# xiaosu-zhu/McQuic

Hardware: AMD Instinct MI355X
Metric: images/sec encode+decode, 768x512 Kodak-shape batch, qp=2 (higher is better)
Workload: dtype f32; 1 GPU; qp=2 reference model Compressor(128, 2, [8192, 2048, 512]), batch=32 768x512 random images per GPU, encode+decode tensor path (BASELINE configs[1]); images_per_gpu=32, parallelism=dp1 (independent image shards, no data-path collective)

## Files before the change

mcquic_amd/csrc/conv_mfma_kernel.h:

```cpp
#pragma once
#include <type_traits>

#include "mcq_common.h"
#include "../../include/mcquic_hip.h"

#ifndef MCQ_PF42A
#define MCQ_PF42A 9
#endif
#ifndef MCQ_PF42B
#define MCQ_PF42B 18
#endif
#ifndef MCQ_PFB
#define MCQ_PFB 18
#endif
#ifndef MCQ_WINO_PERSIST
#define MCQ_WINO_PERSIST 1
#endif
#ifndef MCQ_WINO_PFB2
#define MCQ_WINO_PFB2 48
#endif
#ifndef MCQ_CONV_MAX_MULTI
#define MCQ_CONV_MAX_MULTI 4
#endif

// ... 404 lines not shown
            if constexpr (POST == 2) {
                if (fl & MCQ_CONV_RESIDUAL) {
                    const __amdgpu_buffer_rsrc_t rr = mcq_make_rsrc(mcq_uniform_ptr(P_res + oslab), oslab_bytes);
                    float rv[2][16];
#pragma unroll
                    for (int r = 0; r < 16; ++r) rv[0][r] = mcq_buffer_load_s(rr, pvo, band_so(0, r));
#pragma unroll
                    for (int mb = 0; mb < 4; ++mb) {
                        if (mb < 3) {
#pragma unroll
                            for (int r = 0; r < 16; ++r) rv[(mb + 1) & 1][r] = mcq_buffer_load_s(rr, pvo, band_so(mb + 1, r));
                        }
#pragma unroll
                        for (int r = 0; r < 16; ++r) acc[mb][nb][r] = acc[mb][nb][r] + p.res_scale * rv[mb & 1][r];
                        __builtin_amdgcn_sched_barrier(0);
                    }
                }
            }
            f32x16 sacc[4];
#pragma unroll
            for (int q = 0; q < 4; ++q)
#pragma unroll
                for (int r = 0; r < 16; ++r) sacc[q][r] = mcq_buffer_load_s(pbr, (unsigned)hi * 16u, (unsigned)(q * 32 + mcq_drow(r, 0)) * 4u);
            f32x4v AP[POST_PF];
#pragma unroll
            for (int st = 0; st < POST_PF; ++st) AP[st] = mcq_wload<4>(pwr, pwlane, (unsigned)st * 1024u);
            __builtin_amdgcn_sched_barrier(0);
#pragma unroll
            for (int t = 0; t < POST_STEPS; ++t) {
                float b = acc[t >> 4][nb][t & 15];
                if (POST == 1) b = b * b;
#pragma unroll
                for (int q = 0; q < 4; ++q) sacc[q] = __builtin_amdgcn_mfma_f32_32x32x2f32(AP[t % POST_PF][q], b, sacc[q], 0, 0, 0);
                AP[t % POST_PF] = mcq_wload<4>(pwr, pwlane, (unsigned)(t + POST_PF) * 1024u);
                __builtin_amdgcn_sched_barrier(0);
            }
            if constexpr (POST == 1) {
#pragma unroll
                for (int q = 0; q < 4; ++q) {
                    if (fl & MCQ_CONV_POST_IGDN) {
#pragma unroll
                        for (int r = 0; r < 16; ++r) sacc[q][r] = acc[q][nb][r] * sqrtf(sacc[q][r]);
                    } else {
#pragma unroll
                        for (int r = 0; r < 16; ++r) sacc[q][r] = acc[q][nb][r] * (1.0f / sqrtf(sacc[q][r]));
                    }
#pragma unroll
                    for (int r = 0; r < 16; ++r) mcq_buffer_store_s(sacc[q][r], yr, pvo, band_so(q, r));
                    __builtin_amdgcn_sched_barrier(0);
                }
            } else {
                const __amdgpu_buffer_rsrc_t mr = mcq_make_rsrc(mcq_uniform_ptr(P_mul + oslab), oslab_bytes);
                const __amdgpu_buffer_rsrc_t gr = mcq_make_rsrc(mcq_uniform_ptr(P_gid + oslab), oslab_bytes);
                const __amdgpu_buffer_rsrc_t y2r = mcq_make_rsrc(mcq_uniform_ptr(((fl & MCQ_CONV_DUAL_SILU) ? P_y2 : P_y) + oslab), oslab_bytes);
                float m[2][16], gi[2][16];
#pragma unroll
                for (int r = 0; r < 16; ++r) { m[0][r] = mcq_buffer_load_s(mr, pvo, band_so(0, r)); gi[0][r] = mcq_buffer_load_s(gr, pvo, band_so(0, r)); }
#pragma unroll
                for (int q = 0; q < 4; ++q) {
                    if (q < 3) {
#pragma unroll
                        for (int r = 0; r < 16; ++r) {
                            m[(q + 1) & 1][r] = mcq_buffer_load_s(mr, pvo, band_so(q + 1, r));
                            gi[(q + 1) & 1][r] = mcq_buffer_load_s(gr, pvo, band_so(q + 1, r));
                        }
                    }
#pragma unroll
                    for (int r = 0; r < 16; ++r) sacc[q][r] = m[q & 1][r] * mcq_sigmoid(sacc[q][r]) + gi[q & 1][r];
#pragma unroll
                    for (int r = 0; r < 16; ++r) mcq_buffer_store_s(sacc[q][r], yr, pvo, band_so(q, r));
                    if (fl & MCQ_CONV_DUAL_SILU) {
#pragma unroll
                        for (int r = 0; r < 16; ++r) mcq_buffer_store_s(mcq_silu(sacc[q][r]), y2r, pvo, band_so(q, r));
                    }
                    __builtin_amdgcn_sched_barrier(0);
                }
            }
        }
        return;
    }
    const unsigned fl = p.flags;
    const unsigned HoWo = (unsigned)(p.Ho * p.Wo + tile_zero);
    const unsigned slab_bytes = (unsigned)p.Cout * HoWo * 4u;

    auto epilogue = [&](auto tag, const bool tile_active, auto&& get_acc, const int mb_first, auto count_tag) {
        constexpr unsigned EF = decltype(tag)::value;
        constexpr int MC = decltype(count_tag)::value;
        const unsigned f = EF == RUNTIME_FLAGS ? fl : EF;
        if (!tile_active) return;
        unsigned pvo[NB];
        __amdgpu_buffer_rsrc_t yr[NB], y2r[NB], rr_[NB], mr[NB], gr[NB];
#pragma unroll
        for (int nb = 0; nb < NB; ++nb) {
            const size_t slab = (size_t)img[nb] * p.Cout * HoWo;
            yr[nb] = mcq_make_rsrc(mcq_uniform_ptr(P_y + slab), slab_bytes);
            constexpr unsigned GBWD = MCQ_CONV_GDN_BWD | MCQ_CONV_IGDN_BWD | MCQ_CONV_GATE_BWD;
            if (f & (MCQ_CONV_DUAL_SILU | GBWD)) y2r[nb] = mcq_make_rsrc(mcq_uniform_ptr(P_y2 + slab), slab_bytes);
            if (f & (MCQ_CONV_RESIDUAL | GBWD)) rr_[nb] = mcq_make_rsrc(mcq_uniform_ptr(P_res + slab), slab_bytes);
            if (f & (MCQ_CONV_GDN | MCQ_CONV_IGDN | MCQ_CONV_GATE | MCQ_CONV_MUL | MCQ_CONV_DSILU_MUL | GBWD))
                mr[nb] = mcq_make_rsrc(mcq_uniform_ptr(P_mul + slab), slab_bytes);
            if (f & MCQ_CONV_GATE) gr[nb] = mcq_make_rsrc(mcq_uniform_ptr(P_gid + slab), slab_bytes);
            if (f & MCQ_CONV_SHUFFLE2)
                pvo[nb] = valid[nb] ? ((unsigned)hi * 4u * HoWo + (unsigned)(2 * yo[nb]) * (unsigned)(2 * p.Wo) + (unsigned)(2 * xo[nb])) * 4u
                                    : MCQ_OOB;
            else
                pvo[nb] = valid[nb] ? ((unsigned)(yo[nb] * p.Wo + xo[nb]) + 4u * (unsigned)hi * HoWo) * 4u : MCQ_OOB;
        }
        const __amdgpu_buffer_rsrc_t br = mcq_make_rsrc(mcq_uniform_ptr(P_bias ? P_bias : P_wp), P_bias ? (unsigned)p.Cout * 4u : 0u);

#pragma unroll
        for (int mi = 0; mi < MC; ++mi) {
            const int mb = mb_first + mi;
            const unsigned co_row0 = (unsigned)(co_base + mb * 32);
            float bias16[16];
#pragma unroll
            for (int r = 0; r < 16; ++r)
                bias16[r] = mcq_buffer_load_s(br, (unsigned)hi * 16u, (co_row0 + (unsigned)mcq_drow(r, 0)) * 4u);
            constexpr unsigned SIMPLE = MCQ_CONV_SILU_OUT | MCQ_CONV_RESIDUAL | MCQ_CONV_DUAL_SILU | MCQ_CONV_DSILU_MUL;
            if (EF != RUNTIME_FLAGS && (EF & ~SIMPLE) == 0u && NB <= 2) {
                unsigned sob[16];
#pragma unroll
                for (int r = 0; r < 16; ++r) sob[r] = (co_row0 + (unsigned)mcq_drow(r, 0)) * HoWo * 4u;
                constexpr int EB = OCC >= 3 ? 1 : NB;
#pragma unroll
                for (int nb0 = 0; nb0 < NB; nb0 += EB) {
                    float vv[EB][16], rvv[EB][16], tw[EB][16];
                    if (EF & MCQ_CONV_DSILU_MUL) {
                        if constexpr (PAIR && EB == 2) {
#pragma unroll
                            for (int r = 0; r < 16; ++r) { const f32x2v t2 = mcq_buffer_load2_s(mr[0], pvo[0], sob[r]); tw[0][r] = t2[0]; tw[1][r] = t2[1]; }
                        } else {
#pragma unroll
                        for (int e = 0; e < EB; ++e)
#pragma unroll
                            for (int r = 0; r < 16; ++r) tw[e][r] = mcq_buffer_load_s(mr[nb0 + e], pvo[nb0 + e], sob[r]);
                        }
                    }
                    if (EF & MCQ_CONV_RESIDUAL) {
                        if constexpr (PAIR && EB == 2) {
#pragma unroll
                            for (int r = 0; r < 16; ++r) { const f32x2v t2 = mcq_buffer_load2_s(rr_[0], pvo[0], sob[r]); rvv[0][r] = t2[0]; rvv[1][r] = t2[1]; }
                        } else {
#pragma unroll
                        for (int e = 0; e < EB; ++e)
#pragma unroll
                            for (int r = 0; r < 16; ++r) rvv[e][r] = mcq_buffer_load_s(rr_[nb0 + e], pvo[nb0 + e], sob[r]);
                        }
                    }
#pragma unroll
                    for (int e = 0; e < EB; ++e) {
                        get_acc(mi, nb0 + e, vv[e]);
#pragma unroll
                        for (int r = 0; r < 16; ++r) vv[e][r] = vv[e][r] + bias16[r];
                        if (EF & MCQ_CONV_DSILU_MUL) {
#pragma unroll
                            for (int r = 0; r < 16; ++r) vv[e][r] = vv[e][r] * mcq_dsilu(tw[e][r]);
                        }
                        if (EF & MCQ_CONV_RESIDUAL) {
#pragma unroll
                            for (int r = 0; r < 16; ++r) vv[e][r] = vv[e][r] + p.res_scale * rvv[e][r];
                        }
                        if (EF & MCQ_CONV_SILU_OUT) {
#pragma unroll
                            for (int r = 0; r < 16; ++r) vv[e][r] = mcq_silu(vv[e][r]);
                        }
                        if (EF & MCQ_CONV_DUAL_SILU) {
#pragma unroll
                            for (int r = 0; r < 16; ++r) tw[e][r] = mcq_silu(vv[e][r]);
                        }
                    }
                    if constexpr (PAIR && EB == 2) {
#pragma unroll
                        for (int r = 0; r < 16; ++r) mcq_buffer_store2_s(f32x2v{vv[0][r], vv[1][r]}, yr[0], pvo[0], sob[r]);
                        if (EF & MCQ_CONV_DUAL_SILU) {
#pragma unroll
                            for (int r = 0; r < 16; ++r) mcq_buffer_store2_s(f32x2v{tw[0][r], tw[1][r]}, y2r[0], pvo[0], sob[r]);
                        }
                    } else {
#pragma unroll
                    for (int e = 0; e < EB; ++e) {
#pragma unroll
                        for (int r = 0; r < 16; ++r) mcq_buffer_store_s(vv[e][r], yr[nb0 + e], pvo[nb0 + e], sob[r]);
                        if (EF & MCQ_CONV_DUAL_SILU) {
#pragma unroll
                            for (int r = 0; r < 16; ++r) mcq_buffer_store_s(tw[e][r], y2r[nb0 + e], pvo[nb0 + e], sob[r]);
                        }
                    }
                    }
                }
                continue;
            }
            if constexpr (PAIR) {
                float v0[16], v1[16];
                get_acc(mi, 0, v0);
                get_acc(mi, 1, v1);
#pragma unroll
                for (int r = 0; r < 16; ++r) { v0[r] = v0[r] + bias16[r]; v1[r] = v1[r] + bias16[r]; }
                if (f & MCQ_CONV_SHUFFLE2) {
                    const unsigned W2b = 2u * (unsigned)p.Wo * 4u;
#pragma unroll
                    for (int rq = 0; rq < 4; ++rq) {
                        const unsigned so = ((co_row0 >> 2) + 2u * (unsigned)rq) * HoWo * 16u;
                        f32x4v top = f32x4v{v0[rq * 4 + 0], v0[rq * 4 + 1], v1[rq * 4 + 0], v1[rq * 4 + 1]};
                        f32x4v bot = f32x4v{v0[rq * 4 + 2], v0[rq * 4 + 3], v1[rq * 4 + 2], v1[rq * 4 + 3]};
                        if (f & MCQ_CONV_DSILU_MUL) {
                            const f32x4v mt = mcq_buffer_load4_s(mr[0], pvo[0], so), mb2 = mcq_buffer_load4_s(mr[0], pvo[0], so + W2b);
#pragma unroll
                            for (int e = 0; e < 4; ++e) { top[e] = top[e] * mcq_dsilu(mt[e]); bot[e] = bot[e] * mcq_dsilu(mb2[e]); }
                        }
// ... 89 lines not shown
                    for (int r = 0; r < 16; ++r) {
                        const float sg = mcq_sigmoid(v[r]);
                        mcq_buffer_store_s(g[r] * sg, yr[nb], pvo[nb], so[r]);
                        mcq_buffer_store_s(g[r] * m[r] * sg * (1.0f - sg), y2r[nb], pvo[nb], so[r]);
                    }
                    continue;
                }
                if (f & (MCQ_CONV_GDN | MCQ_CONV_IGDN | MCQ_CONV_GATE | MCQ_CONV_MUL | MCQ_CONV_DSILU_MUL)) {
                    float m[16];
#pragma unroll
                    for (int r = 0; r < 16; ++r) m[r] = mcq_buffer_load_s(mr[nb], pvo[nb], so[r]);
                    if (f & MCQ_CONV_GDN) {
#pragma unroll
                        for (int r = 0; r < 16; ++r) v[r] = m[r] * (1.0f / sqrtf(v[r]));
                    } else if (f & MCQ_CONV_IGDN) {
#pragma unroll
                        for (int r = 0; r < 16; ++r) v[r] = m[r] * sqrtf(v[r]);
                    } else if (f & MCQ_CONV_MUL) {
#pragma unroll
                        for (int r = 0; r < 16; ++r) v[r] = m[r] * v[r];
                    } else if (f & MCQ_CONV_DSILU_MUL) {
#pragma unroll
                        for (int r = 0; r < 16; ++r) v[r] = v[r] * mcq_dsilu(m[r]);
                    } else {
                        float gi[16];
#pragma unroll
                        for (int r = 0; r < 16; ++r) gi[r] = mcq_buffer_load_s(gr[nb], pvo[nb], so[r]);
#pragma unroll
                        for (int r = 0; r < 16; ++r) v[r] = m[r] * mcq_sigmoid(v[r]) + gi[r];
                    }
                }
                if (f & MCQ_CONV_RESIDUAL) {
                    float rv[16];
#pragma unroll
                    for (int r = 0; r < 16; ++r) rv[r] = mcq_buffer_load_s(rr_[nb], pvo[nb], so[r]);
#pragma unroll
                    for (int r = 0; r < 16; ++r) v[r] = v[r] + p.res_scale * rv[r];
                }
                if (f & MCQ_CONV_SILU_OUT) {
#pragma unroll
                    for (int r = 0; r < 16; ++r) v[r] = mcq_silu(v[r]);
                }
#pragma unroll
                for (int r = 0; r < 16; ++r) mcq_buffer_store_s(v[r], yr[nb], pvo[nb], so[r]);
                if (f & MCQ_CONV_DUAL_SILU) {
#pragma unroll
                    for (int r = 0; r < 16; ++r) mcq_buffer_store_s(mcq_silu(v[r]), y2r[nb], pvo[nb], so[r]);
                }
            }
        }
    };
    auto run_epilogue = [&](const bool tile_active, auto&& get_acc, const int mb_first, auto mb_count) {
        const unsigned ef = fl & ~(unsigned)(MCQ_CONV_SILU_IN | MCQ_CONV_SQUARE_IN);
        if (ef == (MCQ_CONV_RESIDUAL | MCQ_CONV_DUAL_SILU))
            epilogue(std::integral_constant<unsigned, MCQ_CONV_RESIDUAL | MCQ_CONV_DUAL_SILU>{}, tile_active, get_acc, mb_first, mb_count);
        else if (ef == MCQ_CONV_SILU_OUT)
            epilogue(std::integral_constant<unsigned, MCQ_CONV_SILU_OUT>{}, tile_active, get_acc, mb_first, mb_count);
        else if (ef == 0u)
            epilogue(std::integral_constant<unsigned, 0u>{}, tile_active, get_acc, mb_first, mb_count);
        else if (ef == MCQ_CONV_RESIDUAL)
            epilogue(std::integral_constant<unsigned, MCQ_CONV_RESIDUAL>{}, tile_active, get_acc, mb_first, mb_count);
        else if (!WINO && TAPS == 9 && NB == 1 && ef == MCQ_CONV_DSILU_MUL)
            epilogue(std::integral_constant<unsigned, MCQ_CONV_DSILU_MUL>{}, tile_active, get_acc, mb_first, mb_count);
        else if (!WINO && TAPS == 9 && NB == 1 && ef == (MCQ_CONV_DSILU_MUL | MCQ_CONV_RESIDUAL))
            epilogue(std::integral_constant<unsigned, MCQ_CONV_DSILU_MUL | MCQ_CONV_RESIDUAL>{}, tile_active, get_acc, mb_first, mb_count);
        else
            epilogue(std::integral_constant<unsigned, RUNTIME_FLAGS>{}, tile_active, get_acc, mb_first, mb_count);
    };

    if constexpr (WASM) {
        const unsigned ef = fl & ~(unsigned)(MCQ_CONV_SILU_IN | MCQ_CONV_SQUARE_IN);
        constexpr unsigned SIMPLE_W = MCQ_CONV_SILU_OUT | MCQ_CONV_RESIDUAL | MCQ_CONV_DUAL_SILU;
        auto wasm_epilogue = [&](auto tag) __attribute__((always_inline)) {
            constexpr unsigned EF = decltype(tag)::value;
            const size_t slab = (size_t)img[0] * p.Cout * HoWo;
            const __amdgpu_buffer_rsrc_t yr = mcq_make_rsrc(mcq_uniform_ptr(P_y + slab), slab_bytes);
            const __amdgpu_buffer_rsrc_t y2r = mcq_make_rsrc(mcq_uniform_ptr((EF & MCQ_CONV_DUAL_SILU) ? P_y2 + slab : P_y + slab), slab_bytes);
            const __amdgpu_buffer_rsrc_t rr = mcq_make_rsrc(mcq_uniform_ptr((EF & MCQ_CONV_RESIDUAL) ? P_res + slab : P_y + slab), slab_bytes);
            const __amdgpu_buffer_rsrc_t br = mcq_make_rsrc(mcq_uniform_ptr(P_bias ? P_bias : P_wp), P_bias ? (unsigned)p.Cout * 4u : 0u);
            unsigned pvo[2];
#pragma unroll
            for (int nb = 0; nb < 2; ++nb)
                pvo[nb] = valid[nb] ? ((unsigned)(yo[nb] * p.Wo + xo[nb]) + 4u * (unsigned)hi * HoWo) * 4u : MCQ_OOB;
            const bool wide = (p.Wo & 1) == 0;
            if constexpr (W2D) {
                unsigned pv4[4];
#pragma unroll
                for (int nb = 0; nb < 4; ++nb)
                    pv4[nb] = valid[nb] ? ((unsigned)(yo[nb] * p.Wo + xo[nb]) + 4u * (unsigned)hi * HoWo) * 4u : MCQ_OOB;
                float bias16[16];
                f32x2v res2[2][16];
#pragma unroll
                for (int r = 0; r < 16; ++r) {
                    const unsigned row = (unsigned)co_base + (unsigned)mcq_drow(r, 0);
                    bias16[r] = mcq_buffer_load_s(br, (unsigned)hi * 16u, row * 4u);
                    if (EF & MCQ_CONV_RESIDUAL) {
#pragma unroll
                        for (int oy = 0; oy < 2; ++oy) {
                            if (wide) res2[oy][r] = mcq_buffer_load2_s(rr, pv4[2 * oy], row * HoWo * 4u);
                            else res2[oy][r] = f32x2v{mcq_buffer_load_s(rr, pv4[2 * oy], row * HoWo * 4u), mcq_buffer_load_s(rr, pv4[2 * oy + 1], row * HoWo * 4u)};
                        }
                    }
                }
#pragma unroll
                for (int r = 0; r < 16; ++r) {
                    if ((r & 3) == 0) __builtin_amdgcn_sched_barrier(0);
// ... 195 lines not shown
```

mcquic_amd/modules/compressor.py:

```python
from __future__ import annotations

import operator
from typing import List, Tuple

import torch
import torch.nn.functional as F
from torch import nn

from ..nn import AttentionBlock, ResidualBlock, ResidualBlockShuffle, ResidualBlockWithStride, conv3x3, pixelShuffle3x3
from ..utils.specification import FileHeader, ImageSize
from .quantizer import BaseQuantizer, ResidualBackwardQuantizer, UMGMQuantizer

from ..utils.specification import VERSION as __version__


_VERSION_OF = operator.attrgetter("_version")
_DATA_PTR_OF = operator.methodcaller("data_ptr")


def _forget_captures_hook(module, incompatible_keys):
    module._forgetCaptures()


class _GraphedCall:
# ... 105 lines not shown
        y = self._encode_latent(x, pad=False)
        yHat, codes, logits = self._quantizer(y, uniforms)
        xHat = self._decoder(yHat)
        return xHat, yHat, codes, logits

    def _trainEncode(self, x: torch.Tensor) -> torch.Tensor:
        y = self._encoder[0](x, dual_silu=True)
        for i in range(1, len(self._encoder)):
            y = self._encoder[i](y)
        return y

    def _repackStale(self):
        convs = self.__dict__.get("_convList")
        if convs is None:
            from ..nn.convs import Conv2d
            convs = self.__dict__["_convList"] = [m for m in self.modules() if isinstance(m, Conv2d)]
        from ..nn.convs import Conv2d
        Conv2d.repack_stale(convs, self.__dict__.get("_packMasks"))
        gdns = self.__dict__.get("_gdnList")
        if gdns is None:
            from ..nn.gdn import GenDivNorm
            gdns = self.__dict__["_gdnList"] = [m for m in self.modules() if isinstance(m, GenDivNorm)]
        if gdns:
            from .. import autograd as AG
            AG.refresh_gdn_operands(gdns)

    def reAssignCodebook(self) -> torch.Tensor:
        return self._quantizer.reAssignCodebook()

    def syncCodebook(self):
        return self._quantizer.syncCodebook()

    @property
    def Codebooks(self):
        return self._quantizer.Codebooks

    @property
    def CDFs(self):
        return self._quantizer.CDFs

    @property
    def NormalizedFreq(self):
        return self._quantizer.NormalizedFreq

    @property
    def CodeUsage(self):
        return torch.cat(list((freq > 1e-6).flatten() for freq in self._quantizer.NormalizedFreq)).float().mean()

    def _check(self, x: torch.Tensor):
        if x.dim() != 4 or x.shape[1] != 3:
            raise RuntimeError(f"expected an image batch [n, 3, h, w], got {tuple(x.shape)}")

    def _encode_latent(self, x: torch.Tensor, pad: bool = True) -> torch.Tensor:
        y = self._encoder[0](self._padding(x) if pad else x, dual_silu=True)
        for i in range(1, len(self._encoder)):
            y = self._encoder[i](y)
        return y

    def encode(self, x: torch.Tensor) -> List[torch.Tensor]:
        self._check(x)
        if x.shape[0] == 0:
            return [c[:0] for c in self.encode(x.new_zeros((1,) + tuple(x.shape[1:])))]
        with torch.no_grad():
            if self._graphs is not None and x.is_cuda and not torch.cuda.is_current_stream_capturing():
                return self._graphed("encode", lambda t: self._quantizer.encode(self._encode_latent(t)), [x.contiguous()])
            return self._quantizer.encode(self._encode_latent(x))

    def decode(self, codes: List[torch.Tensor]) -> torch.Tensor:
        if codes[0].shape[0] == 0:
            return self.decode([c.new_zeros((1,) + tuple(c.shape[1:])) for c in codes])[:0]
        with torch.no_grad():
            if self._graphs is not None and codes[0].is_cuda and not torch.cuda.is_current_stream_capturing():
                return self._graphed("decode", lambda *c: self._decoder(self._quantizer.decode(list(c))), [c.contiguous() for c in codes])
            return self._decoder(self._quantizer.decode(codes))

    def compress(self, x: torch.Tensor) -> Tuple[List[torch.Tensor], List[List[bytes]], List[FileHeader]]:
        self._check(x)
        n, c, h, w = x.shape
        if n == 0:
            return self.encode(x), [], []
        with torch.no_grad():
            codes, binaries, codeSizes = self._quantizer.compress(self._encode_latent(x))
        header = [FileHeader(__version__, self._qp, codeSize, ImageSize(height=h, width=w, channel=c)) for codeSize in codeSizes]
        return codes, binaries, header

    def _checkHeaderGeometry(self, headers: List[FileHeader]):
        for header in headers:
            size, code = header.ImageSize, header.CodeSize
            if not (0 < int(size.height) <= (1 << 20) and 0 < int(size.width) <= (1 << 20)):
                raise RuntimeError("The header's image size is out of range.")
            base = self._padding._base
            ph, pw = -(-int(size.height) // base) * base, -(-int(size.width) // base) * base
            if len(code.heights) < 1 or int(code.heights[0]) * 16 != ph or int(code.widths[0]) * 16 != pw:
                raise RuntimeError(f"The header's code size {list(code.heights)} x {list(code.widths)} does not belong to a "
                                   f"{size.height} x {size.width} image.")

    def decompress(self, binaries: List[List[bytes]], headers: List[FileHeader]) -> torch.Tensor:
        if type(self)._encode_latent is BaseCompressor._encode_latent:
            self._checkHeaderGeometry(headers)
        with torch.no_grad():
            restored = self._decoder(self._quantizer.decompress(binaries, [header.CodeSize for header in headers]))
        imageSize = headers[0].ImageSize
        H, W = restored.shape[-2], restored.shape[-1]
        h, w = imageSize.height, imageSize.width
        cropTop, cropLeft = (H - h) // 2, (W - w) // 2
        return restored[..., cropTop:cropTop + h, cropLeft:cropLeft + w]


class Compressor(BaseCompressor):
    def __init__(self, channel: int, m: int, k: List[int], permutationRate: float = 0.0):
        encoder = nn.Sequential(
            conv3x3(3, channel, 2),
            ResidualBlock(channel, channel),
            ResidualBlockWithStride(channel, channel),
            AttentionBlock(channel),
            ResidualBlock(channel, channel),
            ResidualBlockWithStride(channel, channel),
            ResidualBlock(channel, channel))
        decoder = nn.Sequential(
            ResidualBlock(channel, channel),
            ResidualBlockShuffle(channel, channel),
            AttentionBlock(channel),
            ResidualBlock(channel, channel),
            ResidualBlockShuffle(channel, channel),
            ResidualBlock(channel, channel),
            pixelShuffle3x3(channel, 3, 2))
        quantizer = UMGMQuantizer(channel, m, k, permutationRate, {
            "latentStageEncoder": lambda: nn.Sequential(
                ResidualBlockWithStride(channel, channel), ResidualBlock(channel, channel), AttentionBlock(channel)),
            "quantizationHead": lambda: nn.Sequential(
                ResidualBlock(channel, channel), AttentionBlock(channel), conv3x3(channel, channel)),
            "latentHead": lambda: nn.Sequential(
                ResidualBlock(channel, channel), AttentionBlock(channel), conv3x3(channel, channel)),
            "restoreHead": lambda: nn.Sequential(
                AttentionBlock(channel), ResidualBlock(channel, channel), ResidualBlockShuffle(channel, channel)),
            "dequantizationHead": lambda: nn.Sequential(
                AttentionBlock(channel), conv3x3(channel, channel), ResidualBlock(channel, channel)),
            "sideHead": lambda: nn.Sequential(
                AttentionBlock(channel), conv3x3(channel, channel), ResidualBlock(channel, channel)),
        })
        super().__init__(encoder, quantizer, decoder)



class Neon(BaseCompressor):

    def __init__(self, channel: int, k: int, size: List[int], denseNorm: bool = False, *_, **__):
        quantizer = ResidualBackwardQuantizer(k, size, denseNorm)
        q = quantizer.channel
        encoder = nn.Sequential(
            conv3x3(3, channel),
            AttentionBlock(channel, 32, denseNorm),
            ResidualBlock(channel, channel, 32, denseNorm),
            ResidualBlock(channel, channel, 32, denseNorm),
# ... 43 lines not shown
```

mcquic_amd/modules/quantizer.py:

```python
from __future__ import annotations

import math
from typing import Callable, Dict, List, Optional, Union

import torch
from torch import nn

from .. import ops
from .entropyCoder import EntropyCoder, VariousMCoder

EPS = 1e-6
_TORCH_RAND = __import__("os").environ.get("MCQUIC_AMD_TORCH_RAND", "0") == "1"


class _CodebookCache:

    def __init__(self):
        self._packed: Optional[ops.PackedCodebook] = None
        self._key = None

    def invalidate(self):
        self._packed, self._key = None, None

    def get(self, codebook: torch.Tensor) -> ops.PackedCodebook:
# ... 82 lines not shown
            return deq, code, logit
        logit = ops.vq_logits(x, cb, self._temperature, float(EPS))
        code, index, hot = ops.vq_gumbel_sample(logit, uniforms[0], uniforms[1], freqEMA, exponent, rng, counts)
        return (index, hot), code, logit


class _multiCodebookDeQuantization(nn.Module):

    def __init__(self, codebook: nn.Parameter, cache: _CodebookCache):
        super().__init__()
        self._m, self._k, self._d = codebook.shape
        self._codebook = codebook
        self._cache = [cache]

    def forward(self, sample) -> torch.Tensor:
        if torch.is_tensor(sample):
            return sample
        index, hot = sample
        return ops.vq_dequant_soft(index, hot, self._cache[0].get(self._codebook))

    def decode(self, code: torch.Tensor, dual_silu: bool = False) -> torch.Tensor:
        return ops.vq_gather(code, self._cache[0].get(self._codebook), dual_silu=dual_silu)


class _quantizerEncoder(nn.Module):

    def __init__(self, quantizer, dequantizer, latentStageEncoder, quantizationHead, latentHead):
        super().__init__()
        self._quantizer = quantizer
        self._dequantizer = dequantizer
        self._latentStageEncoder = latentStageEncoder
        self._quantizationHead = quantizationHead
        self._latentHead = latentHead

    @property
    def Codebook(self):
        return self._quantizer._codebook

    def syncCodebook(self):
        self._quantizer.syncCodebook()

    def reAssignCodebook(self, freq: torch.Tensor) -> torch.Tensor:
        return self._quantizer.reAssignCodebook(freq)

    def encode(self, x: torch.Tensor):
        residual, code, _ = self._encode(x)
        return residual, code

    def _encode(self, x: torch.Tensor):
        from ..nn import blocks
        z = self._latentStageEncoder(x)
        head = self._latentHead
        if head is None:
            qin = self._quantizationHead(z)
            return None, self._quantizer.encode(qin), qin
        if blocks.lockstep_ok([self._quantizationHead, head], [z, z]):
            last = len(head) - 1
            q, t = blocks.lockstep_infer([self._quantizationHead, head], [z, z], layers=last)
            qin = self._quantizationHead[last](q)
            code = self._quantizer.encode(qin)
        else:
            qin = self._quantizationHead(z)
            code = self._quantizer.encode(qin)
            t = z
            for i in range(len(head) - 1):
                t = head[i](t)
        deq = self._dequantizer.decode(code)
        return head[len(head) - 1](t, res=deq, res_scale=-1.0, dual_silu=True), code, qin


    def _forward(self, x: torch.Tensor, freqEMA: torch.Tensor, uniforms=None, step=None):
        z = self._latentStageEncoder(x)
        if self._latentHead is None:
            q, code, logit = self._quantizer(self._quantizationHead(z), freqEMA, uniforms, step)
            return q, None, code, logit
        head = self._latentHead
        if torch.is_grad_enabled():
            from .. import autograd as AG
            hz, qin = AG.lockstep([head, self._quantizationHead], [z, z])
            q, code, logit = self._quantizer(qin, freqEMA, uniforms, step)
            residual, q = AG.sub_pass(hz, self._dequantizer(q))
            return q, residual, code, logit
        q, code, logit = self._quantizer(self._quantizationHead(z), freqEMA, uniforms, step)
        deq = self._dequantizer(q)
        t = z
        for i in range(len(head) - 1):
            t = head[i](t)
        return q, head[len(head) - 1](t, res=deq, res_scale=-1.0, dual_silu=True), code, logit

    def forward(self, x: torch.Tensor, freqEMA: torch.Tensor, uniforms=None, step=None):
        return self._forward(x, freqEMA, uniforms, step)


class _quantizerDecoder(nn.Module):

    def __init__(self, dequantizer, dequantizationHead, sideHead, restoreHead):
        super().__init__()
        self._dequantizer = dequantizer
        self._dequantizationHead = dequantizationHead
        self._sideHead = sideHead
        self._restoreHead = restoreHead

    def decode(self, code: torch.Tensor, formerLevel: Optional[torch.Tensor]):
        from ..nn import blocks
        deq = self._dequantizer.decode(code, dual_silu=True)
        if self._sideHead is None:
            return self._restoreHead(self._dequantizationHead(deq))
        if blocks.lockstep_ok([self._dequantizationHead, self._sideHead], [deq, formerLevel]):
            q, side = blocks.lockstep_infer([self._dequantizationHead, self._sideHead], [deq, formerLevel])
        else:
            q, side = self._dequantizationHead(deq), self._sideHead(formerLevel)
        return self._restoreHead(ops.add(q, side, dual_silu=True))


    def forward(self, q, formerLevel: Optional[torch.Tensor]):
        if self._sideHead is not None and torch.is_grad_enabled():
            from .. import autograd as AG
            x, side = AG.lockstep([self._dequantizationHead, self._sideHead], [self._dequantizer(q), formerLevel])
            return self._restoreHead(AG.add(x, side, dual_silu=True))
        from ..nn import blocks
        x = blocks.run_stack(self._dequantizationHead, self._dequantizer(q))
        if self._sideHead is not None:
            if torch.is_grad_enabled():
                from .. import autograd as AG
                x = AG.add(x, self._sideHead(formerLevel), dual_silu=True)
            else:
                x = ops.add(x, self._sideHead(formerLevel), dual_silu=True)
        return self._restoreHead(x)


class BaseQuantizer(nn.Module):

    def __init__(self, m: int, k: List[int]):
        super().__init__()
        self._entropyCoder = EntropyCoder(m, k)
        self._m = m
        self._k = k

    @property
    def CDFs(self):
        return self._entropyCoder.CDFs

    @property
    def NormalizedFreq(self):
        return self._entropyCoder.NormalizedFreq

    def _stepPrologue(self, x: torch.Tensor, uniforms):
        if not x.is_cuda:
            raise NotImplementedError(f"mcquic_amd: the training forward of {type(self).__name__} runs on a HIP device only (input on "
                                      f"{x.device}); there is no CPU / PyTorch fallback -- move the model and the batch to cuda")
        coder = self._entropyCoder
        want_rng = uniforms is None and not _TORCH_RAND
        return ops.vq_step_prologue(list(coder._freqEMA), EPS, want_rng, coder.countBuffer(x.device))

    def compress(self, x: torch.Tensor):
        codes = self.encode(x)
        binaries, codeSize = self._entropyCoder.compress(codes)
        return codes, binaries, codeSize

    def decompress(self, binaries, codeSize) -> torch.Tensor:
        return self.decode(self._entropyCoder.decompress(binaries, codeSize))


class UMGMQuantizer(BaseQuantizer):
# ... 310 lines not shown
```

mcquic_amd/nn/blocks.py:

```python
from __future__ import annotations

import os
from typing import Dict, Optional

import torch
from torch import nn

from .. import autograd as AG
from .. import ops
from .convs import conv1x1, conv3x3, pixelShuffle3x3
from .gdn import GenDivNorm, InvGenDivNorm

__all__ = ["ResidualBlockWithStride", "ResidualBlockShuffle", "ResidualBlock", "AttentionBlock"]

_BRANCH_STREAMS = os.environ.get("MCQUIC_AMD_BRANCH_STREAMS", "1") != "0"
_NORM_NODES = os.environ.get("MCQUIC_AMD_NORM_NODES", "1") != "0"
_BLOCK_NODES = os.environ.get("MCQUIC_AMD_BLOCK_NODES", "1") != "0"
_side_streams: Dict[tuple, "torch.cuda.Stream"] = {}
_MULTI_MAX_PIXELS = int(os.environ.get("MCQUIC_AMD_MULTI_MAX_PIXELS", str(64 * 1024)))
_FORK_MIN_PIXELS = int(os.environ.get("MCQUIC_AMD_FORK_MIN_PIXELS", str(128 * 1024)))


def _side_stream(main: "torch.cuda.Stream") -> "torch.cuda.Stream":
    key = (main.device.index, main.cuda_stream)
# ... 4 lines not shown


class _fork:

    def __init__(self, x: torch.Tensor):
        self.on = _BRANCH_STREAMS and x.is_cuda and x.shape[0] * x.shape[-2] * x.shape[-1] >= _FORK_MIN_PIXELS
        if self.on:
            self.main = torch.cuda.current_stream(x.device)
            self.side = _side_stream(self.main)
        self.ctx = None

    def __enter__(self):
        if self.on:
            self.side.wait_stream(self.main)
            self.ctx = torch.cuda.stream(self.side)
            self.ctx.__enter__()
        return self

    def __exit__(self, *exc):
        if self.ctx is not None:
            self.ctx.__exit__(*exc)
        return False

    def join(self, t: torch.Tensor) -> torch.Tensor:
        if self.on:
            self.main.wait_stream(self.side)
            t.record_stream(self.main)
        return t


class _residulBlock(nn.Module):

    def __init__(self, act1: nn.Module, conv1: nn.Module, act2: nn.Module, conv2: nn.Module, skip: Optional[nn.Module]):
        super().__init__()
        self._branch = nn.Sequential(act1, conv1, act2, conv2)
        self._skip = skip


class GroupNorm(nn.GroupNorm):

    def forward(self, x: torch.Tensor) -> torch.Tensor:
        if self.training and torch.is_grad_enabled():
            return AG.group_norm(x, self)
        return ops.group_norm(x, self.weight, self.bias, self.num_groups, self.eps)


class ResidualBlock(_residulBlock):

    def __init__(self, inChannels: int, outChannels: int, groups: int = 1, denseNorm: bool = False):
        super().__init__(nn.SiLU(), conv3x3(inChannels, outChannels), GroupNorm(groups, outChannels) if denseNorm else nn.SiLU(),
                         conv3x3(outChannels, outChannels), conv1x1(inChannels, outChannels) if inChannels != outChannels else None)
        self.denseNorm = bool(denseNorm)

    def forward(self, x: torch.Tensor, res2: Optional[torch.Tensor] = None) -> torch.Tensor:
        if self.training and torch.is_grad_enabled():
            if self._skip is None and (_NORM_NODES or not self.denseNorm):
                return AG.residual_block(x, self)
            sx, x = AG.silu_fork(x)
            t = self._branch[1](sx)
            t = self._branch[2](t) if self.denseNorm else AG.silu(t)
            return self._branch[3](t, res=x if self._skip is None else self._skip(x), dual_silu=True)
        if self.denseNorm:
            t = self._branch[2](self._branch[1](x, silu_in=True))
        else:
            t = self._branch[1](x, silu_in=True, silu_out=True)
        identity = x if self._skip is None else self._skip(x)
        return self._branch[3](t, res=identity, dual_silu=True)


class ResidualBlockWithStride(_residulBlock):

    def __init__(self, inChannels: int, outChannels: int, stride: int = 2, groups: int = 1, denseNorm: bool = False):
        if stride != 2:
            raise NotImplementedError("only stride-2 ResidualBlockWithStride is on the path")
        super().__init__(nn.SiLU(), conv3x3(inChannels, outChannels, stride=stride), GenDivNorm(outChannels),
                         conv3x3(outChannels, outChannels), conv3x3(inChannels, outChannels, stride=stride))

    def forward(self, x: torch.Tensor) -> torch.Tensor:
        if self.training and torch.is_grad_enabled():
            if _BLOCK_NODES and self._branch[1].bias is not None:
                return AG.scale_block(x, self, up=False)
            sx, x = AG.silu_fork(x)
            t = self._branch[2](self._branch[1](sx))
            return self._branch[3](t, res=self._skip(x), dual_silu=True)
        with _fork(x) as f:
            identity = self._skip(x)
        c1, gdn = self._branch[1], self._branch[2]
        fuse = ops.post_ok(x, c1.packed(), c1.stride, "gdn")
        if fuse:
            t = c1(x, silu_in=True, post_gdn=gdn.packed_post(), tile=0 if fuse == 1 else fuse)
        else:
            t = gdn(c1(x, silu_in=True))
        return self._branch[3](t, res=f.join(identity), dual_silu=True)


class ResidualBlockShuffle(_residulBlock):

    def __init__(self, inChannels: int, outChannels: int, upsample: int = 2, groups: int = 1, denseNorm: bool = False):
        if upsample != 2:
            raise NotImplementedError("only 2x ResidualBlockShuffle is on the path")
        super().__init__(nn.SiLU(), pixelShuffle3x3(inChannels, outChannels, upsample), InvGenDivNorm(outChannels),
                         conv3x3(outChannels, outChannels), pixelShuffle3x3(inChannels, outChannels, upsample))

    def forward(self, x: torch.Tensor) -> torch.Tensor:
        if self.training and torch.is_grad_enabled():
            if _BLOCK_NODES and self._branch[1][0].bias is not None:
                return AG.scale_block(x, self, up=True)
            sx, x = AG.silu_fork(x)
            t = self._branch[2](self._branch[1](sx))
            return self._branch[3](t, res=self._skip(x), dual_silu=True)
        with _fork(x) as f:
            identity = self._skip(x)
        up, igdn = self._branch[1][0], self._branch[2]
        fuse = ops.post_ok(x, up.packed(), 1, "igdn", shuffle2=True)
        if fuse:
            t = ops.conv2d(x, up.packed_subpixel(), 1, silu_in=True, shuffle2=True, post_igdn=igdn.packed_post(), tile=0 if fuse == 1 else fuse)
        else:
            t = igdn(self._branch[1](x, silu_in=True))
        return self._branch[3](t, res=f.join(identity), dual_silu=True)


class AttentionBlock(nn.Module):

    def __init__(self, channel: int, groups: int = 1, denseNorm: bool = False):
        super().__init__()
        self._mainBranch = nn.Sequential(*[ResidualBlock(channel, channel, groups, denseNorm) for _ in range(3)])
        self._sideBranch = nn.Sequential(*[ResidualBlock(channel, channel, groups, denseNorm) for _ in range(3)],
                                         conv1x1(channel, channel))
        self.denseNorm = bool(denseNorm)

    def forward(self, x: torch.Tensor) -> torch.Tensor:
        if self.training and torch.is_grad_enabled():
            if self.denseNorm and not _NORM_NODES:
                xa, xb, xc = AG.fork(x, 3)
                return AG.gate(self._mainBranch(xa), self._sideBranch(xb), xc)
            return AG.attention_block(x, self)
        if ops._MULTI and not self.denseNorm and x.shape[0] * x.shape[2] * x.shape[3] <= _MULTI_MAX_PIXELS:
            return _attn_infer_multi([self], [x])[0]
        last, gate = self._sideBranch[2], self._sideBranch[3]
        fuse = 0 if (self.denseNorm or last._skip is not None) else ops.post_ok(x, last._branch[3].packed(), 1, "gate")
        if fuse:
            with _fork(x) as f:
                b = x
                for i in range(2):
                    b = self._sideBranch[i](b)
                t = last._branch[1](b, silu_in=True, silu_out=True)
            a = self._mainBranch(x)
            f.join(b)
            return ops.conv2d(f.join(t), last._branch[3].packed(), 1, res=b, post_gate=gate.packed_post(), gate_mul=a, gate_id=x, dual_silu=True, tile=0 if fuse == 1 else fuse)
        with _fork(x) as f:
            b = x
            for i in range(3):
                b = self._sideBranch[i](b)
        a = self._mainBranch(x)
        return self._sideBranch[3](f.join(b), gate_mul=a, gate_id=x, dual_silu=True)


def run_stack(stack, x: torch.Tensor) -> torch.Tensor:
    mods = list(stack)
    for i, m in enumerate(mods):
        nxt = mods[i + 1] if i + 1 < len(mods) else None
        if type(m).__name__ == "Conv2d" and isinstance(nxt, (_residulBlock, AttentionBlock)) and m.training and torch.is_grad_enabled():
            x = m(x, dual_silu=True)
        else:
            x = m(x)
    return x


def lockstep_ok(stacks, xs) -> bool:
    if not (ops._MULTI and len(stacks) >= 2 and AG.lockstep_compatible(stacks)):
        return False
    if any(x.shape != xs[0].shape for x in xs[1:]):
        return False
    return xs[0].shape[0] * xs[0].shape[2] * xs[0].shape[3] <= _MULTI_MAX_PIXELS


def _rb_infer_multi(blocks, xs):
    ts = ops.conv2d_multi(xs, [blk._branch[1].packed() for blk in blocks], silu_in=True, silu_out=True)
    return ops.conv2d_multi(ts, [blk._branch[3].packed() for blk in blocks], per_problem=[dict(res=x) for x in xs], dual_silu=True)


def _attn_infer_multi(layer, xs):
    k = len(layer)
    a, b = list(xs), list(xs)
    for i in range(3):
        ys = _rb_infer_multi([m._mainBranch[i] for m in layer] + [m._sideBranch[i] for m in layer], a + b)
        a, b = ys[:k], ys[k:]
    return ops.conv2d_multi(b, [m._sideBranch[3].packed() for m in layer],
                            per_problem=[dict(gate_mul=ai, gate_id=xi) for ai, xi in zip(a, xs)], dual_silu=True)


def lockstep_infer(stacks, xs, layers: Optional[int] = None):
    xs = list(xs)
    for li, layer in enumerate(zip(*stacks)):
        if layers is not None and li >= layers:
            break
        kind = AG.lockstep_kind(layer[0])
        if kind == "conv":
            xs = ops.conv2d_multi(xs, [m.packed() for m in layer], dual_silu=True)
            continue
        twins = [ops.silu_twin(x) is not None for x in xs]
        if any(twins) and not all(twins):
            for x, has in zip(xs, twins):
                if not has:
                    ops.set_silu_twin(x, ops.silu(x))
        xs = (_rb_infer_multi if kind == "rb" else _attn_infer_multi)(list(layer), xs)
    return xs
```

Measured before the change: 255.3 images/s.

## Skip unused SiLU twin outputs and specialize gate epilogue at compile time

Adds a twin flag through the residual and attention blocks and the stack runners. The dual SiLU output tensor is now written only when the next module actually reads it, which removes redundant full-tensor stores at stack ends and before plain convs. The kernel also gets a compile-time specialised gate epilogue for 1x1 non-Winograd convs, and the persistent gate path is templated on the twin flag. The cost is more template instantiations, and any consumer that still expects a twin where none is produced would break.

New measurement: 256.7 images/s, median of 6. About the same (+0.5%).

```diff
diff --git a/mcquic_amd/csrc/conv_mfma_kernel.h b/mcquic_amd/csrc/conv_mfma_kernel.h
--- a/mcquic_amd/csrc/conv_mfma_kernel.h
+++ b/mcquic_amd/csrc/conv_mfma_kernel.h
@@ -480,29 +480,34 @@
             } else {
                 const __amdgpu_buffer_rsrc_t mr = mcq_make_rsrc(mcq_uniform_ptr(P_mul + oslab), oslab_bytes);
                 const __amdgpu_buffer_rsrc_t gr = mcq_make_rsrc(mcq_uniform_ptr(P_gid + oslab), oslab_bytes);
-                const __amdgpu_buffer_rsrc_t y2r = mcq_make_rsrc(mcq_uniform_ptr(((fl & MCQ_CONV_DUAL_SILU) ? P_y2 : P_y) + oslab), oslab_bytes);
-                float m[2][16], gi[2][16];
-#pragma unroll
-                for (int r = 0; r < 16; ++r) { m[0][r] = mcq_buffer_load_s(mr, pvo, band_so(0, r)); gi[0][r] = mcq_buffer_load_s(gr, pvo, band_so(0, r)); }
-#pragma unroll
-                for (int q = 0; q < 4; ++q) {
-                    if (q < 3) {
-#pragma unroll
-                        for (int r = 0; r < 16; ++r) {
-                            m[(q + 1) & 1][r] = mcq_buffer_load_s(mr, pvo, band_so(q + 1, r));
-                            gi[(q + 1) & 1][r] = mcq_buffer_load_s(gr, pvo, band_so(q + 1, r));
-                        }
-                    }
-#pragma unroll
-                    for (int r = 0; r < 16; ++r) sacc[q][r] = m[q & 1][r] * mcq_sigmoid(sacc[q][r]) + gi[q & 1][r];
-#pragma unroll
-                    for (int r = 0; r < 16; ++r) mcq_buffer_store_s(sacc[q][r], yr, pvo, band_so(q, r));
-                    if (fl & MCQ_CONV_DUAL_SILU) {
-#pragma unroll
-                        for (int r = 0; r < 16; ++r) mcq_buffer_store_s(mcq_silu(sacc[q][r]), y2r, pvo, band_so(q, r));
-                    }
-                    __builtin_amdgcn_sched_barrier(0);
-                }
+                auto close_gate = [&](auto twin_tag) __attribute__((always_inline)) {
+                    constexpr bool TWIN = decltype(twin_tag)::value;
+                    const __amdgpu_buffer_rsrc_t y2r = mcq_make_rsrc(mcq_uniform_ptr((TWIN ? P_y2 : P_y) + oslab), oslab_bytes);
+                    float m[2][16], gi[2][16];
+#pragma unroll
+                    for (int r = 0; r < 16; ++r) { m[0][r] = mcq_buffer_load_s(mr, pvo, band_so(0, r)); gi[0][r] = mcq_buffer_load_s(gr, pvo, band_so(0, r)); }
+#pragma unroll
+                    for (int q = 0; q < 4; ++q) {
+                        if (q < 3) {
+#pragma unroll
+                            for (int r = 0; r < 16; ++r) {
+                                m[(q + 1) & 1][r] = mcq_buffer_load_s(mr, pvo, band_so(q + 1, r));
+                                gi[(q + 1) & 1][r] = mcq_buffer_load_s(gr, pvo, band_so(q + 1, r));
+                            }
+                        }
+#pragma unroll
+                        for (int r = 0; r < 16; ++r) sacc[q][r] = m[q & 1][r] * mcq_sigmoid(sacc[q][r]) + gi[q & 1][r];
+#pragma unroll
+                        for (int r = 0; r < 16; ++r) mcq_buffer_store_s(sacc[q][r], yr, pvo, band_so(q, r));
+                        if constexpr (TWIN) {
+#pragma unroll
+                            for (int r = 0; r < 16; ++r) mcq_buffer_store_s(mcq_silu(sacc[q][r]), y2r, pvo, band_so(q, r));
+                        }
+                        __builtin_amdgcn_sched_barrier(0);
+                    }
+                };
+                if (fl & MCQ_CONV_DUAL_SILU) close_gate(std::true_type{});
+                else close_gate(std::false_type{});
             }
         }
         return;
@@ -545,7 +550,7 @@
             for (int r = 0; r < 16; ++r)
                 bias16[r] = mcq_buffer_load_s(br, (unsigned)hi * 16u, (co_row0 + (unsigned)mcq_drow(r, 0)) * 4u);
             constexpr unsigned SIMPLE = MCQ_CONV_SILU_OUT | MCQ_CONV_RESIDUAL | MCQ_CONV_DUAL_SILU | MCQ_CONV_DSILU_MUL;
-            if (EF != RUNTIME_FLAGS && (EF & ~SIMPLE) == 0u && NB <= 2) {
+            if (EF != RUNTIME_FLAGS && ((EF & ~SIMPLE) == 0u || EF == MCQ_CONV_GATE) && NB <= 2) {
                 unsigned sob[16];
 #pragma unroll
                 for (int r = 0; r < 16; ++r) sob[r] = (co_row0 + (unsigned)mcq_drow(r, 0)) * HoWo * 4u;
@@ -564,6 +569,15 @@
                             for (int r = 0; r < 16; ++r) tw[e][r] = mcq_buffer_load_s(mr[nb0 + e], pvo[nb0 + e], sob[r]);
                         }
                     }
+                    if (EF == MCQ_CONV_GATE) {
+#pragma unroll
+                        for (int e = 0; e < EB; ++e)
+#pragma unroll
+                            for (int r = 0; r < 16; ++r) {
+                                tw[e][r] = mcq_buffer_load_s(mr[nb0 + e], pvo[nb0 + e], sob[r]);
+                                rvv[e][r] = mcq_buffer_load_s(gr[nb0 + e], pvo[nb0 + e], sob[r]);
+                            }
+                    }
                     if (EF & MCQ_CONV_RESIDUAL) {
                         if constexpr (PAIR && EB == 2) {
 #pragma unroll
@@ -583,6 +597,10 @@
                         if (EF & MCQ_CONV_DSILU_MUL) {
 #pragma unroll
                             for (int r = 0; r < 16; ++r) vv[e][r] = vv[e][r] * mcq_dsilu(tw[e][r]);
+                        }
+                        if (EF == MCQ_CONV_GATE) {
+#pragma unroll
+                            for (int r = 0; r < 16; ++r) vv[e][r] = tw[e][r] * mcq_sigmoid(vv[e][r]) + rvv[e][r];
                         }
                         if (EF & MCQ_CONV_RESIDUAL) {
 #pragma unroll
@@ -778,6 +796,12 @@
     };
     auto run_epilogue = [&](const bool tile_active, auto&& get_acc, const int mb_first, auto mb_count) {
         const unsigned ef = fl & ~(unsigned)(MCQ_CONV_SILU_IN | MCQ_CONV_SQUARE_IN);
+        if constexpr (!WINO && TAPS == 1 && PRO == PRO_NONE && !PAIR && NB == 1) {
+            if (ef == MCQ_CONV_GATE) {
+                epilogue(std::integral_constant<unsigned, MCQ_CONV_GATE>{}, tile_active, get_acc, mb_first, mb_count);
+                return;
+            }
+        }
         if (ef == (MCQ_CONV_RESIDUAL | MCQ_CONV_DUAL_SILU))
             epilogue(std::integral_constant<unsigned, MCQ_CONV_RESIDUAL | MCQ_CONV_DUAL_SILU>{}, tile_active, get_acc, mb_first, mb_count);
         else if (ef == MCQ_CONV_SILU_OUT)
diff --git a/mcquic_amd/modules/compressor.py b/mcquic_amd/modules/compressor.py
--- a/mcquic_amd/modules/compressor.py
+++ b/mcquic_amd/modules/compressor.py
@@ -181,10 +181,13 @@
             raise RuntimeError(f"expected an image batch [n, 3, h, w], got {tuple(x.shape)}")
 
     def _encode_latent(self, x: torch.Tensor, pad: bool = True) -> torch.Tensor:
+        from ..nn import blocks
         y = self._encoder[0](self._padding(x) if pad else x, dual_silu=True)
-        for i in range(1, len(self._encoder)):
-            y = self._encoder[i](y)
-        return y
+        return blocks.infer_stack(list(self._encoder)[1:], y)
+
+    def _decode_latent(self, yHat: torch.Tensor) -> torch.Tensor:
+        from ..nn import blocks
+        return blocks.infer_stack(self._decoder, yHat)
 
     def encode(self, x: torch.Tensor) -> List[torch.Tensor]:
         self._check(x)
@@ -200,8 +203,8 @@
             return self.decode([c.new_zeros((1,) + tuple(c.shape[1:])) for c in codes])[:0]
         with torch.no_grad():
             if self._graphs is not None and codes[0].is_cuda and not torch.cuda.is_current_stream_capturing():
-                return self._graphed("decode", lambda *c: self._decoder(self._quantizer.decode(list(c))), [c.contiguous() for c in codes])
-            return self._decoder(self._quantizer.decode(codes))
+                return self._graphed("decode", lambda *c: self._decode_latent(self._quantizer.decode(list(c))), [c.contiguous() for c in codes])
+            return self._decode_latent(self._quantizer.decode(codes))
 
     def compress(self, x: torch.Tensor) -> Tuple[List[torch.Tensor], List[List[bytes]], List[FileHeader]]:
         self._check(x)
@@ -228,7 +231,7 @@
         if type(self)._encode_latent is BaseCompressor._encode_latent:
             self._checkHeaderGeometry(headers)
         with torch.no_grad():
-            restored = self._decoder(self._quantizer.decompress(binaries, [header.CodeSize for header in headers]))
+            restored = self._decode_latent(self._quantizer.decompress(binaries, [header.CodeSize for header in headers]))
         imageSize = headers[0].ImageSize
         H, W = restored.shape[-2], restored.shape[-1]
         h, w = imageSize.height, imageSize.width
diff --git a/mcquic_amd/modules/quantizer.py b/mcquic_amd/modules/quantizer.py
--- a/mcquic_amd/modules/quantizer.py
+++ b/mcquic_amd/modules/quantizer.py
@@ -158,7 +158,7 @@
         z = self._latentStageEncoder(x)
         head = self._latentHead
         if head is None:
-            qin = self._quantizationHead(z)
+            qin = blocks.infer_stack(self._quantizationHead, z)
             return None, self._quantizer.encode(qin), qin
         if blocks.lockstep_ok([self._quantizationHead, head], [z, z]):
             last = len(head) - 1
@@ -166,11 +166,9 @@
             qin = self._quantizationHead[last](q)
             code = self._quantizer.encode(qin)
         else:
-            qin = self._quantizationHead(z)
+            qin = blocks.infer_stack(self._quantizationHead, z)
             code = self._quantizer.encode(qin)
-            t = z
-            for i in range(len(head) - 1):
-                t = head[i](t)
+            t = blocks.infer_stack(list(head)[:-1], z, twin=False)
         deq = self._dequantizer.decode(code)
         return head[len(head) - 1](t, res=deq, res_scale=-1.0, dual_silu=True), code, qin
 
@@ -213,9 +211,9 @@
         if self._sideHead is None:
             return self._restoreHead(self._dequantizationHead(deq))
         if blocks.lockstep_ok([self._dequantizationHead, self._sideHead], [deq, formerLevel]):
-            q, side = blocks.lockstep_infer([self._dequantizationHead, self._sideHead], [deq, formerLevel])
+            q, side = blocks.lockstep_infer([self._dequantizationHead, self._sideHead], [deq, formerLevel], twin=False)
         else:
-            q, side = self._dequantizationHead(deq), self._sideHead(formerLevel)
+            q, side = blocks.infer_stack(self._dequantizationHead, deq, twin=False), blocks.infer_stack(self._sideHead, formerLevel, twin=False)
         return self._restoreHead(ops.add(q, side, dual_silu=True))
 
 
diff --git a/mcquic_amd/nn/blocks.py b/mcquic_amd/nn/blocks.py
--- a/mcquic_amd/nn/blocks.py
+++ b/mcquic_amd/nn/blocks.py
@@ -80,7 +80,7 @@
                          conv3x3(outChannels, outChannels), conv1x1(inChannels, outChannels) if inChannels != outChannels else None)
         self.denseNorm = bool(denseNorm)
 
-    def forward(self, x: torch.Tensor, res2: Optional[torch.Tensor] = None) -> torch.Tensor:
+    def forward(self, x: torch.Tensor, res2: Optional[torch.Tensor] = None, twin: bool = True) -> torch.Tensor:
         if self.training and torch.is_grad_enabled():
             if self._skip is None and (_NORM_NODES or not self.denseNorm):
                 return AG.residual_block(x, self)
@@ -93,7 +93,7 @@
         else:
             t = self._branch[1](x, silu_in=True, silu_out=True)
         identity = x if self._skip is None else self._skip(x)
-        return self._branch[3](t, res=identity, dual_silu=True)
+        return self._branch[3](t, res=identity, dual_silu=twin)
 
 
 class ResidualBlockWithStride(_residulBlock):
@@ -104,7 +104,7 @@
         super().__init__(nn.SiLU(), conv3x3(inChannels, outChannels, stride=stride), GenDivNorm(outChannels),
                          conv3x3(outChannels, outChannels), conv3x3(inChannels, outChannels, stride=stride))
 
-    def forward(self, x: torch.Tensor) -> torch.Tensor:
+    def forward(self, x: torch.Tensor, twin: bool = True) -> torch.Tensor:
         if self.training and torch.is_grad_enabled():
             if _BLOCK_NODES and self._branch[1].bias is not None:
                 return AG.scale_block(x, self, up=False)
@@ -119,7 +119,7 @@
             t = c1(x, silu_in=True, post_gdn=gdn.packed_post(), tile=0 if fuse == 1 else fuse)
         else:
             t = gdn(c1(x, silu_in=True))
-        return self._branch[3](t, res=f.join(identity), dual_silu=True)
+        return self._branch[3](t, res=f.join(identity), dual_silu=twin)
 
 
 class ResidualBlockShuffle(_residulBlock):
@@ -130,7 +130,7 @@
         super().__init__(nn.SiLU(), pixelShuffle3x3(inChannels, outChannels, upsample), InvGenDivNorm(outChannels),
                          conv3x3(outChannels, outChannels), pixelShuffle3x3(inChannels, outChannels, upsample))
 
-    def forward(self, x: torch.Tensor) -> torch.Tensor:
+    def forward(self, x: torch.Tensor, twin: bool = True) -> torch.Tensor:
         if self.training and torch.is_grad_enabled():
             if _BLOCK_NODES and self._branch[1][0].bias is not None:
                 return AG.scale_block(x, self, up=True)
@@ -145,7 +145,7 @@
             t = ops.conv2d(x, up.packed_subpixel(), 1, silu_in=True, shuffle2=True, post_igdn=igdn.packed_post(), tile=0 if fuse == 1 else fuse)
         else:
             t = igdn(self._branch[1](x, silu_in=True))
-        return self._branch[3](t, res=f.join(identity), dual_silu=True)
+        return self._branch[3](t, res=f.join(identity), dual_silu=twin)
 
 
 class AttentionBlock(nn.Module):
@@ -157,14 +157,14 @@
                                          conv1x1(channel, channel))
         self.denseNorm = bool(denseNorm)
 
-    def forward(self, x: torch.Tensor) -> torch.Tensor:
+    def forward(self, x: torch.Tensor, twin: bool = True) -> torch.Tensor:
         if self.training and torch.is_grad_enabled():
             if self.denseNorm and not _NORM_NODES:
                 xa, xb, xc = AG.fork(x, 3)
                 return AG.gate(self._mainBranch(xa), self._sideBranch(xb), xc)
             return AG.attention_block(x, self)
         if ops._MULTI and not self.denseNorm and x.shape[0] * x.shape[2] * x.shape[3] <= _MULTI_MAX_PIXELS:
-            return _attn_infer_multi([self], [x])[0]
+            return _attn_infer_multi([self], [x], twin=twin)[0]
         last, gate = self._sideBranch[2], self._sideBranch[3]
         fuse = 0 if (self.denseNorm or last._skip is not None) else ops.post_ok(x, last._branch[3].packed(), 1, "gate")
         if fuse:
@@ -173,15 +173,19 @@
                 for i in range(2):
                     b = self._sideBranch[i](b)
                 t = last._branch[1](b, silu_in=True, silu_out=True)
-            a = self._mainBranch(x)
+            a = self._stack(self._mainBranch, x)
             f.join(b)
-            return ops.conv2d(f.join(t), last._branch[3].packed(), 1, res=b, post_gate=gate.packed_post(), gate_mul=a, gate_id=x, dual_silu=True, tile=0 if fuse == 1 else fuse)
+            return ops.conv2d(f.join(t), last._branch[3].packed(), 1, res=b, post_gate=gate.packed_post(), gate_mul=a, gate_id=x, dual_silu=twin, tile=0 if fuse == 1 else fuse)
         with _fork(x) as f:
-            b = x
-            for i in range(3):
-                b = self._sideBranch[i](b)
-        a = self._mainBranch(x)
-        return self._sideBranch[3](f.join(b), gate_mul=a, gate_id=x, dual_silu=True)
+            b = self._stack(self._sideBranch, x)
+        a = self._stack(self._mainBranch, x)
+        return self._sideBranch[3](f.join(b), gate_mul=a, gate_id=x, dual_silu=twin)
+
+    @staticmethod
+    def _stack(branch, x: torch.Tensor) -> torch.Tensor:
+        for i in range(3):
+            x = branch[i](x, twin=i < 2)
+        return x
 
 
 def run_stack(stack, x: torch.Tensor) -> torch.Tensor:
@@ -203,34 +207,50 @@
     return xs[0].shape[0] * xs[0].shape[2] * xs[0].shape[3] <= _MULTI_MAX_PIXELS
 
 
-def _rb_infer_multi(blocks, xs):
+def _rb_infer_multi(blocks, xs, twin: bool = True):
     ts = ops.conv2d_multi(xs, [blk._branch[1].packed() for blk in blocks], silu_in=True, silu_out=True)
-    return ops.conv2d_multi(ts, [blk._branch[3].packed() for blk in blocks], per_problem=[dict(res=x) for x in xs], dual_silu=True)
-
-
-def _attn_infer_multi(layer, xs):
+    return ops.conv2d_multi(ts, [blk._branch[3].packed() for blk in blocks], per_problem=[dict(res=x) for x in xs], dual_silu=twin)
+
+
+def _attn_infer_multi(layer, xs, twin: bool = True):
     k = len(layer)
     a, b = list(xs), list(xs)
     for i in range(3):
-        ys = _rb_infer_multi([m._mainBranch[i] for m in layer] + [m._sideBranch[i] for m in layer], a + b)
+        ys = _rb_infer_multi([m._mainBranch[i] for m in layer] + [m._sideBranch[i] for m in layer], a + b, twin=i < 2)
         a, b = ys[:k], ys[k:]
     return ops.conv2d_multi(b, [m._sideBranch[3].packed() for m in layer],
-                            per_problem=[dict(gate_mul=ai, gate_id=xi) for ai, xi in zip(a, xs)], dual_silu=True)
-
-
-def lockstep_infer(stacks, xs, layers: Optional[int] = None):
+                            per_problem=[dict(gate_mul=ai, gate_id=xi) for ai, xi in zip(a, xs)], dual_silu=twin)
+
+
+def reads_twin(module) -> bool:
+    return isinstance(module, (_residulBlock, AttentionBlock))
+
+
+def infer_stack(stack, x: torch.Tensor, twin: bool = True) -> torch.Tensor:
+    mods = list(stack)
+    for i, m in enumerate(mods):
+        if reads_twin(m) and not (m.training and torch.is_grad_enabled()):
+            x = m(x, twin=reads_twin(mods[i + 1]) if i + 1 < len(mods) else twin)
+        else:
+            x = m(x)
+    return x
+
+
+def lockstep_infer(stacks, xs, layers: Optional[int] = None, twin: bool = True):
     xs = list(xs)
+    first = list(stacks[0])
     for li, layer in enumerate(zip(*stacks)):
         if layers is not None and li >= layers:
             break
         kind = AG.lockstep_kind(layer[0])
+        out_twin = reads_twin(first[li + 1]) if li + 1 < len(first) else twin
         if kind == "conv":
-            xs = ops.conv2d_multi(xs, [m.packed() for m in layer], dual_silu=True)
+            xs = ops.conv2d_multi(xs, [m.packed() for m in layer], dual_silu=out_twin)
             continue
         twins = [ops.silu_twin(x) is not None for x in xs]
         if any(twins) and not all(twins):
             for x, has in zip(xs, twins):
                 if not has:
                     ops.set_silu_twin(x, ops.silu(x))
-        xs = (_rb_infer_multi if kind == "rb" else _attn_infer_multi)(list(layer), xs)
+        xs = (_rb_infer_multi if kind == "rb" else _attn_infer_multi)(list(layer), xs, twin=out_twin)
     return xs
```
